# Alisah-Ozcan/HEonGPU

Measured on AMD Instinct MI355X. Metric: homomorphic mults/sec (CKKS N=2^16, L=16) + NTT GB/s vs HBM roofline, higher is better.
Workload: dtype u64

## Files before the change

### heongpu_amd/csrc/ntt.hip

```cpp
#include "ntt.hpp"
#define HEGPU_FP_TU ntt
#include "fpmod.cuh"

namespace hegpu {

#define NTT_THREADS 256

#ifdef NTT_ABLATION_HEADER
#include NTT_ABLATION_HEADER
#else
__device__ __forceinline__ u64 gld(const u64* p) { return *p; }
__device__ __forceinline__ void gst(u64* p, u64 v) { *p = v; }
#define NTT_ABLATE_BFLY(x, y, w)
#define NTT_ABLATE_FPBFLY(x, y, w)
#define NTT_ABLATE_TW(load, root0, s) (load)
#define NTT_FP_TW(t, i, c) ((t)[i])
#endif

__device__ __forceinline__ u64 csub(u64 x, u64 m) { return (x >= m) ? x - m : x; }

typedef unsigned long long u64x2_t __attribute__((ext_vector_type(2)));
struct ConstTw {
    const u64x2_t __attribute__((address_space(4)))* p;
    __device__ __forceinline__ ulonglong2 operator[](u32 i) const
    {
        const u64x2_t v = p[i];
        return make_ulonglong2(v.x, v.y);
    }
};
__device__ __forceinline__ ConstTw const_tw(const ulonglong2* t)
{
#pragma clang diagnostic push
#pragma clang diagnostic ignored "-Wold-style-cast"
    return ConstTw{(const u64x2_t __attribute__((address_space(4)))*) reinterpret_cast<const u64x2_t*>(t)};
#pragma clang diagnostic pop
}

__device__ __forceinline__ int ld_const_i32(const int* p)
{
#pragma clang diagnostic push
#pragma clang diagnostic ignored "-Wold-style-cast"
    return *(const int __attribute__((address_space(4)))*) p;
#pragma clang diagnostic pop
}
__device__ __forceinline__ Mod ld_const_mod(const Mod* p)
{
#pragma clang diagnostic push
#pragma clang diagnostic ignored "-Wold-style-cast"
    const u64 __attribute__((address_space(4)))* w = (const u64 __attribute__((address_space(4)))*) reinterpret_cast<const u64*>(p);
#pragma clang diagnostic pop
    static_assert(sizeof(Mod) == 56, "seven words");
    Mod m;
    m.q = w[0];
// ... 244 lines not shown
#pragma unroll
    for (int j = 0; j < half; j++) {
        u64 s = x[j] + x[j + half];
        u64 d = x[j] + c.q4 - x[j + half];
        x[j] = shoup_full(s, ninv, c);
        x[j + half] = shoup_full(d, w1ninv, c);
    }
}

struct PolySel {
    u64 in_off, out_off;
    int mod;
    int digit;
    int item, j;
};

__device__ __forceinline__ int udiv16(int x, unsigned magic)
{
    return magic ? (int) __umulhi((unsigned) x, magic) : x;
}

__device__ __forceinline__ PolySel select_poly(const NttArgs& a, int poly)
{
    PolySel s;
    if (a.group_span) {
        const int k = udiv16(poly, a.mg_group_span), r = poly - k * a.group_span;
        if (a.polys_per_item) {
            const int per_item = udiv16(a.polys_per_item, a.mg_mod_count);
            const int it = udiv16(r, a.mg_per_item), d = r - it * per_item;
            poly = it * a.polys_per_item + d * a.mod_count + k;
        } else {
            poly = r * a.mod_count + k;
        }
    }
    int item = 0, j = poly;
    if (a.polys_per_item) {
        item = udiv16(poly, a.mg_polys_per_item);
        j = poly - item * a.polys_per_item;
    }
    int k = j - udiv16(j, a.mg_mod_count) * a.mod_count;
    if (a.mod_order) k = a.mod_order[k];
    s.mod = a.mod_offset + k;
    u64 slot = a.poly_order ? (u64) a.poly_order[j] : (u64) j;
    s.digit = a.decomp_mods ? udiv16(j, a.mg_decomp_mods) : -1;
    u64 in_slot = a.decomp_mods ? (u64) s.digit * (a.decomp_in_mul ? a.decomp_in_mul : 1) + a.decomp_in_add : slot;
    if (a.decomp_out_mul) slot = (u64) s.digit * a.decomp_out_mul + (u64) (j - s.digit * a.decomp_mods);
    s.in_off = (u64) item * a.in_item_stride + (in_slot << a.n_power);
    s.out_off = (u64) item * a.out_item_stride + (slot << a.n_power);
    s.item = item;
    s.j = j;
    return s;
}

__device__ __forceinline__ int col_phys(int e) { return e ^ (((e >> 8) & 1) << 4); }
__device__ __forceinline__ int row_phys(int e) { return e ^ (((e >> 5) & 7) << 1); }

__device__ __forceinline__ void wave_lds_fence()
{
    __builtin_amdgcn_fence(__ATOMIC_RELEASE, "wavefront");
    __builtin_amdgcn_wave_barrier();
    __builtin_amdgcn_fence(__ATOMIC_ACQUIRE, "wavefront");
}

#define COL_LDS_ELEMS 4096
#define ROW_LDS_ELEMS 4096

__device__ __forceinline__ bool fwd_stages_lazy(const Mod& md, u64 lazy_q_max) { return md.q <= lazy_q_max; }
#define NTT_ROW_LAZY_MAX_Q 0x0666666666666666ull
__device__ __forceinline__ bool row_stages_lazy(const Mod& md, u64 lazy_q_max) { return md.q <= lazy_q_max || md.q <= NTT_ROW_LAZY_MAX_Q; }

template <int S1, bool DECOMP, bool LAZY, bool SREG = false>
__device__ __forceinline__ void fwd_col_body(const NttArgs& a, const PolySel& ps, const Mod& md, u64* lds,
                                             const u64* sreg = nullptr)
{
    constexpr int R = 1 << S1;
    constexpr int CT = 4096 / R;
    constexpr int NSA = S1 - 4;
    constexpr int RA = 1 << NSA;
    constexpr int G = 16 / RA;
    const int t = threadIdx.x;
    const QC qc = make_qc(md.q);
    const ulonglong2* __restrict__ tw = a.tw + ((u64) ps.mod << a.n_power);
    const u64* __restrict__ src = a.in + ps.in_off + blockIdx.x * CT;
    u64* __restrict__ dst = a.out + ps.out_off + blockIdx.x * CT;

    const u64 half_qP = a.half_on ? a.mods[a.half_src_mod].q : 0;
    const u64 half_hm = a.half_on ? a.half_mod[ps.mod] : 0;
    u64 x[16];
    const int col = t % CT, r1 = t / CT;
    u64 v[16];
    if constexpr (NSA > 0) {
#pragma unroll
        for (int g = 0; g < G; g++) {
            const int L = t + NTT_THREADS * g;
            const int c = L % CT, rb = L / CT;
#pragma unroll
            for (int k = 0; k < RA; k++) v[g * RA + k] = SREG ? sreg[g * RA + k] : gld(&src[(u64) (rb + 16 * k) * 256 + c]);
        }
    } else {
#pragma unroll
        for (int k = 0; k < 16; k++) v[k] = SREG ? sreg[k] : gld(&src[(u64) k * 256 + col]);
    }
    if (DECOMP && a.half_on) {
#pragma unroll
        for (int k = 0; k < 16; k++) v[k] = sub_mod(reduce64(add_mod(v[k], a.half, half_qP), md), half_hm, md.q);
    } else if (DECOMP && !LAZY && a.mods[ps.digit].q > 8 * md.q) {
#pragma unroll
        for (int k = 0; k < 16; k++) v[k] = reduce64(v[k], md);
// ... 167 lines not shown
    const u64* __restrict__ ks = ep.ks + ep.ks_item_stride * ps.item + ((u64) (part * ep.ks_part_limbs + limb) << a.n_power) + e0;
    const u64 off = ((u64) (part * ep.limbs + limb) << a.n_power);
    const bool with_ct = ep.ct && (!ep.ct_parts || part < ep.ct_parts);
    const u64* ct = with_ct ? ep.ct + ep.ct_item_stride * ps.item + off + e0 : nullptr;
    u64* out = ep.out + ep.out_item_stride * ps.item + off;
    const u64 inv = ep.inv[ps.mod];
#pragma unroll
    for (int h = 0; h < 2; h++) {
        u64 kv[8], cv[8];
#pragma unroll
        for (int k = 0; k < 8; k++) kv[k] = ks[16 * (8 * h + k)];
        if (with_ct) {
#pragma unroll
            for (int k = 0; k < 8; k++) cv[k] = ct[16 * (8 * h + k)];
        }
        u64 r[8];
#pragma unroll
        for (int k = 0; k < 8; k++)
            r[k] = mul_barrett(sub_mod(kv[k], lds[row_phys(row * 256 + i0 + 16 * (8 * h + k))], md.q), inv, md);
        if (with_ct) {
#pragma unroll
            for (int k = 0; k < 8; k++) r[k] = add_mod(cv[k], r[k], md.q);
        }
        if (ep.galois_inv) {
#pragma unroll
            for (int k = 0; k < 8; k++) {
                const u32 e = (u32) e0 + 16 * (8 * h + k);
                const u32 ex = ((2u * (__brev(e) >> (32 - a.n_power)) + 1u) * ep.galois_inv) & ((2u << a.n_power) - 1u);
                out[__brev((ex - 1u) >> 1) >> (32 - a.n_power)] = r[k];
            }
        } else {
#pragma unroll
            for (int k = 0; k < 8; k++) out[e0 + 16 * (8 * h + k)] = r[k];
        }
    }
}

template <bool LAZY>
__device__ __forceinline__ void fwd_row_body(const NttArgs& a, const PolySel& ps, const Mod& md, u64* lds)
{
    const int t = threadIdx.x;
    const QC qc = make_qc(md.q);
    const int s1 = a.n_power - 8;
    const ulonglong2* __restrict__ tw = a.tw + ((u64) ps.mod << a.n_power);
    u64* __restrict__ p = a.out + ps.out_off + (u64) blockIdx.x * 4096;

    const int row = t >> 4, i0 = t & 15;
    const u32 crow = blockIdx.x * 16 + row;
    u64 x[16];
#pragma unroll
    for (int k = 0; k < 16; k++) x[k] = gld(&p[row * 256 + i0 + 16 * k]);
    ct_radix<4, LAZY>(x, tw, (1u << s1) + crow, qc);
#pragma unroll
    for (int k = 0; k < 16; k++) lds[row_phys(row * 256 + i0 + 16 * k)] = x[k];
    wave_lds_fence();
#pragma unroll
    for (int k = 0; k < 8; k++) {
        ulonglong2 v = *reinterpret_cast<const ulonglong2*>(&lds[row_phys(row * 256 + 16 * i0 + 2 * k)]);
        x[2 * k] = v.x;
        x[2 * k + 1] = v.y;
    }
    ct_radix16_tb<LAZY>(x, a.twB + ((u64) ps.mod * (15u << (a.n_power - 4))) + ((u64) crow * 15 * 16 + i0), qc);
    if (LAZY) {
#pragma unroll
        for (int k = 0; k < 16; k++) x[k] = reduce64(x[k], md);
    } else {
#pragma unroll
        for (int k = 0; k < 16; k++) x[k] = csub(csub(csub(x[k], qc.q4), 2 * qc.q), qc.q);
    }
    wave_lds_fence();
#pragma unroll
    for (int k = 0; k < 8; k++)
        *reinterpret_cast<ulonglong2*>(&lds[row_phys(row * 256 + 16 * i0 + 2 * k)]) =
            make_ulonglong2(x[2 * k], x[2 * k + 1]);
    wave_lds_fence();
    row_store_all(a, ps, md, a.out + ps.out_off, (u64) blockIdx.x * 4096 + row * 256 + i0, lds, row, i0);
}

__device__ __forceinline__ void fwd_row_body_fp(const NttArgs& a, const PolySel& ps, const Mod& md, u64* lds)
{
    const int t = threadIdx.x;
    const FC fc = make_fc(md.q, FP_SITE(FPS_FWD_ROW, a.n_power - 12));
    const int s1 = a.n_power - 8;
    const ulonglong2* __restrict__ tw = a.tw + ((u64) ps.mod << a.n_power);
    u64* __restrict__ p = a.out + ps.out_off + (u64) blockIdx.x * 4096;

    const int row = t >> 4, i0 = t & 15;
    const u32 crow = blockIdx.x * 16 + row;
    double x[16];
#pragma unroll
    for (int k = 0; k < 16; k++) x[k] = as_f64(p[row * 256 + i0 + 16 * k]);
    fp_ct_radix<4>(x, tw, (1u << s1) + crow, fc, 0u, true);
#pragma unroll
    for (int k = 0; k < 16; k++) lds[row_phys(row * 256 + i0 + 16 * k)] = as_bits(x[k]);
    wave_lds_fence();
#pragma unroll
    for (int k = 0; k < 8; k++) {
        ulonglong2 v = *reinterpret_cast<const ulonglong2*>(&lds[row_phys(row * 256 + 16 * i0 + 2 * k)]);
        x[2 * k] = as_f64(v.x);
        x[2 * k + 1] = as_f64(v.y);
    }
    fp_ct_radix16_tb8(x, a.twB8 + ((u64) ps.mod * (15u << (a.n_power - 4))) + ((u64) crow * 15 * 16 + i0), fc);
    wave_lds_fence();
#pragma unroll
    for (int k = 0; k < 8; k++)
        *reinterpret_cast<ulonglong2*>(&lds[row_phys(row * 256 + 16 * i0 + 2 * k)]) =
            make_ulonglong2(fp_to_u64(x[2 * k]), fp_to_u64(x[2 * k + 1]));
    wave_lds_fence();
    row_store_all(a, ps, md, a.out + ps.out_off, (u64) blockIdx.x * 4096 + row * 256 + i0, lds, row, i0);
}

__global__ __launch_bounds__(NTT_THREADS) void ntt_fwd_row(NttArgs a)
{
    __shared__ __attribute__((aligned(16))) u64 lds[ROW_LDS_ELEMS];
    const PolySel ps = select_poly(a, blockIdx.y);
    if (a.skip_identity && ps.mod == ps.digit) return;
    const Mod md = a.mods[ps.mod];
    if (md.fp) fwd_row_body_fp(a, ps, md, lds);
    else if (row_stages_lazy(md, a.lazy_q_max)) fwd_row_body<true>(a, ps, md, lds);
    else fwd_row_body<false>(a, ps, md, lds);
}

template <int S1>
__device__ __forceinline__ int single_pos(int row, int col)
{
    return (row >> 4) * 4096 + row_phys((row & 15) * 256 + col);
}

template <int S1, bool FP, bool LAZY, bool DECOMP = false>
__device__ __forceinline__ void fwd_single_body(const NttArgs& a, const PolySel& ps, const Mod& md, u64* limb)
{
    constexpr int R = 1 << S1;
    constexpr int CT = 4096 / R;
    constexpr int NSA = S1 - 4;
    constexpr int RA = 1 << NSA;
    constexpr int G = 16 / RA;
    const int t = threadIdx.x, g = t >> 8, tt = t & 255;
    const QC qc = make_qc(md.q);
    const FC fc = make_fc(md.q, FP_SITE(FPS_FWD_SINGLE, S1 - 4));
    const ulonglong2* __restrict__ tw = a.tw + ((u64) ps.mod << a.n_power);
    const u64* __restrict__ src = a.in + ps.in_off + g * CT;
    const int col = tt % CT, r1 = tt / CT;
    u64 dv[DECOMP ? 16 : 1];
    double dy[(DECOMP && FP) ? 16 : 1];
    if constexpr (DECOMP) {
        if constexpr (NSA > 0) {
#pragma unroll
// ... 64 lines not shown
        } else {
#pragma unroll
            for (int k = 0; k < 16; k++) {
                if constexpr (DECOMP) x[k] = dy[k];
                else x[k] = fp_from_u64(src[(u64) k * 256 + col]);
            }
        }
        fp_ct_radix<4>(x, tw, (u32) (RA + r1), fc, FpColSched<S1>::b_before, FpColSched<S1>::b_at_end);
#pragma unroll
        for (int k = 0; k < 16; k++) limb[single_pos<S1>(16 * r1 + k, g * CT + col)] = as_bits(x[k]);
    } else {
        u64 x[16];
        if constexpr (NSA > 0) {
#pragma unroll
            for (int gi = 0; gi < G; gi++) {
                const int L = tt + 256 * gi;
                const int c = L % CT, rb = L / CT;
                u64 y[RA];
#pragma unroll
                for (int k = 0; k < RA; k++) {
                    if constexpr (DECOMP) y[k] = dv[gi * RA + k];
                    else y[k] = gld(&src[(u64) (rb + 16 * k) * 256 + c]);
                }
                ct_radix<NSA, LAZY>(y, tw, 1u, qc);
#pragma unroll
                for (int k = 0; k < RA; k++) limb[single_pos<S1>(rb + 16 * k, g * CT + c)] = y[k];
            }
            __syncthreads();
#pragma unroll
            for (int k = 0; k < 16; k++) x[k] = limb[single_pos<S1>(16 * r1 + k, g * CT + col)];
        } else {
#pragma unroll
            for (int k = 0; k < 16; k++) {
                if constexpr (DECOMP) x[k] = dv[k];
                else x[k] = src[(u64) k * 256 + col];
            }
        }
        ct_radix<4, LAZY>(x, tw, (u32) (RA + r1), qc);
#pragma unroll
        for (int k = 0; k < 16; k++) limb[single_pos<S1>(16 * r1 + k, g * CT + col)] = x[k];
    }
    __syncthreads();
    u64* lds = limb + g * 4096;
    const int row = tt >> 4, i0 = tt & 15;
    const u32 crow = g * 16 + row;
    const ulonglong2* __restrict__ tb = a.twB + ((u64) ps.mod * (15u << (a.n_power - 4))) + ((u64) crow * 15 * 16 + i0);
    u64 r[16];
    if constexpr (FP) {
        double x[16];
#pragma unroll
        for (int k = 0; k < 16; k++) x[k] = as_f64(lds[row_phys(row * 256 + i0 + 16 * k)]);
        fp_ct_radix<4>(x, tw, (1u << S1) + crow, fc, 0u, true);
#pragma unroll
        for (int k = 0; k < 16; k++) lds[row_phys(row * 256 + i0 + 16 * k)] = as_bits(x[k]);
        wave_lds_fence();
#pragma unroll
        for (int k = 0; k < 8; k++) {
            ulonglong2 v = *reinterpret_cast<const ulonglong2*>(&lds[row_phys(row * 256 + 16 * i0 + 2 * k)]);
            x[2 * k] = as_f64(v.x);
            x[2 * k + 1] = as_f64(v.y);
        }
        fp_ct_radix16_tb8(x, a.twB8 + ((u64) ps.mod * (15u << (a.n_power - 4))) + ((u64) crow * 15 * 16 + i0), fc);
#pragma unroll
        for (int k = 0; k < 16; k++) r[k] = fp_to_u64(x[k]);
    } else {
        u64 x[16];
#pragma unroll
        for (int k = 0; k < 16; k++) x[k] = lds[row_phys(row * 256 + i0 + 16 * k)];
        ct_radix<4, LAZY>(x, tw, (1u << S1) + crow, qc);
#pragma unroll
        for (int k = 0; k < 16; k++) lds[row_phys(row * 256 + i0 + 16 * k)] = x[k];
        wave_lds_fence();
#pragma unroll
        for (int k = 0; k < 8; k++) {
            ulonglong2 v = *reinterpret_cast<const ulonglong2*>(&lds[row_phys(row * 256 + 16 * i0 + 2 * k)]);
            x[2 * k] = v.x;
            x[2 * k + 1] = v.y;
        }
        ct_radix16_tb<LAZY>(x, tb, qc);
        if (LAZY) {
#pragma unroll
            for (int k = 0; k < 16; k++) r[k] = reduce64(x[k], md);
        } else {
#pragma unroll
            for (int k = 0; k < 16; k++) r[k] = csub(csub(csub(x[k], qc.q4), 2 * qc.q), qc.q);
        }
    }
    wave_lds_fence();
#pragma unroll
    for (int k = 0; k < 8; k++)
        *reinterpret_cast<ulonglong2*>(&lds[row_phys(row * 256 + 16 * i0 + 2 * k)]) = make_ulonglong2(r[2 * k], r[2 * k + 1]);
    wave_lds_fence();
    row_store_all(a, ps, md, a.out + ps.out_off, (u64) g * 4096 + row * 256 + i0, lds, row, i0);
}

template <int S1, bool DECOMP = false>
__global__ __launch_bounds__(16 << S1, 4) void ntt_fwd_single(NttArgs a)
{
    extern __shared__ __attribute__((aligned(16))) u64 limb[];
    const PolySel ps = select_poly(a, blockIdx.x);
    if (DECOMP && a.skip_identity && ps.mod == ps.digit) return;
    const Mod md = a.mods[ps.mod];
    if (md.fp) fwd_single_body<S1, true, false, DECOMP>(a, ps, md, limb);
    else if (fwd_stages_lazy(md, a.lazy_q_max)) fwd_single_body<S1, false, true, DECOMP>(a, ps, md, limb);
    else fwd_single_body<S1, false, false, DECOMP>(a, ps, md, limb);
}

__device__ __forceinline__ void acc128(u64& hi, u64& lo, u64 a, u64 b)
{
    u64 h, l;
    mul64wide(a, b, h, l);
    lo += l;
    hi += h + (lo < l);
}

template <bool LAZY>
__device__ __forceinline__ void ks_row_digit(u64 (&x)[16], const u64* __restrict__ p, u64* lds,
                                             const ulonglong2* twa, const ulonglong2* __restrict__ tb,
                                             const QC& qc, const Mod& md, int row, int i0)
{
#pragma unroll
    for (int k = 0; k < 16; k++) x[k] = gld(&p[row * 256 + i0 + 16 * k]);
#pragma unroll
    for (int s = 0; s < 4; s++) {
        const int half = 8 >> s;
#pragma unroll
        for (int b = 0; b < (1 << s); b++) {
            const ulonglong2 w = twa[((1 << s) - 1 + b) * 16 + row];
#pragma unroll
            for (int j = 0; j < half; j++) ct_bfly<LAZY>(x[b * 2 * half + j], x[b * 2 * half + j + half], w, qc);
        }
    }
#pragma unroll
    for (int k = 0; k < 16; k++) lds[row_phys(row * 256 + i0 + 16 * k)] = x[k];
    wave_lds_fence();
#pragma unroll
    for (int k = 0; k < 8; k++) {
        ulonglong2 v = *reinterpret_cast<const ulonglong2*>(&lds[row_phys(row * 256 + 16 * i0 + 2 * k)]);
        x[2 * k] = v.x;
        x[2 * k + 1] = v.y;
    }
    ct_radix16_tb<LAZY>(x, tb, qc);
    if (!LAZY) {
#pragma unroll
        for (int k = 0; k < 16; k++) x[k] = csub(csub(csub(x[k], qc.q4), 2 * qc.q), qc.q);
    }
    wave_lds_fence();
#pragma unroll
    for (int k = 0; k < 8; k++)
        *reinterpret_cast<ulonglong2*>(&lds[row_phys(row * 256 + 16 * i0 + 2 * k)]) =
            make_ulonglong2(x[2 * k], x[2 * k + 1]);
    wave_lds_fence();
#pragma unroll
    for (int k = 0; k < 16; k++) x[k] = lds[row_phys(row * 256 + i0 + 16 * k)];
    wave_lds_fence();
}

struct KsIdx { int item, tile, slot; bool valid; int d0, d1; };
__host__ __device__ __forceinline__ unsigned ks_slots(const KsMacArgs& a, int kind)
{
    const int all = a.slot_count ? a.slot_count : a.rc;
    if (a.int_slot_count <= 0 || kind == 0) return (unsigned) all;
    return kind == 1 ? (unsigned) a.int_slot_count : (unsigned) (all - a.int_slot_count);
}
template <bool SPLIT, int KIND = 0>
__device__ __forceinline__ KsIdx ks_index(const KsMacArgs& a)
{
    const unsigned b = blockIdx.x, xcd = b & 7u, j = b >> 3;
    const unsigned splits = SPLIT ? (unsigned) a.splits : 1u;
    const unsigned units = (unsigned) a.items * splits;
    const unsigned tiles = 1u << (a.n_power - 12);
    const unsigned total = ks_slots(a, KIND) * tiles * units, chunk = (total + 7u) >> 3;
    const unsigned lin = xcd * chunk + j;
    const unsigned g = lin / units, unit = lin - g * units;
    const unsigned item = SPLIT ? unit / splits : unit, sp = SPLIT ? unit - item * splits : 0u;
    const unsigned nslots = ks_slots(a, KIND), gt = g / nslots;
    KsIdx r;
    r.valid = lin < total;
    r.item = (int) item;
    r.tile = (int) gt;
    int si = (int) (g - gt * nslots);
    if (KIND == 1 && a.int_slot_count > 0) {
        si = a.int_slots[r.valid ? si : 0];
    } else {
        si += a.slot_first;
        if (KIND == 2 && a.int_slot_count > 0) {
#pragma unroll
// ... 103 lines not shown
            acc0[k] = reduce128(h0[k], l0[k], md);
            acc1[k] = reduce128(h1[k], l1[k], md);
        }
        int tt = threadIdx.x;
        asm volatile("" : "+v"(tt));
        const int trow = tt >> 4, ti0 = tt & 15;
        const u64 e0 = (u64) tile_s * 4096 + trow * 256 + ti0;
        const u64 inv = a.tail.inv[midx_s];
        const bool lazy_t = row_stages_lazy(md, a.lazy_q_max);
        const ulonglong2* __restrict__ ttb = a.twB + ((u64) midx_s * (15u << (a.n_power - 4))) + ((u64) (tile_s * 16 + trow) * 15 * 16 + ti0);
        auto part = [&](int p, const u64 (&acc)[16]) {
            u64 cv[16], x[16];
            const bool with_ct = ks_tail_ct(a, item_s, slot_s, p, e0, cv);
            const u64* pT = ks_tail_T(a, item_s, slot_s, tile_s, p);
            if (lazy_t) {
                ks_row_digit<true>(x, pT, lds, twa, ttb, qc, md, trow, ti0);
#pragma unroll
                for (int k = 0; k < 16; k++) x[k] = reduce64(x[k], md);
            } else {
                ks_row_digit<false>(x, pT, lds, twa, ttb, qc, md, trow, ti0);
            }
            ks_tail_store(a, item_s, slot_s, p, e0, md, inv, acc, x, with_ct, cv);
        };
        __builtin_amdgcn_sched_barrier(0);
        part(0, acc0);
        __builtin_amdgcn_sched_barrier(0);
        part(1, acc1);
        return;
    }
    u64* po = (SPLIT ? const_cast<u64*>(pin) + dig_off * ki.d0 - (u64) tile * 4096
                     : a.out + a.out_item_stride * item + ((u64) slot << a.n_power)) +
              (u64) tile * 4096 + row * 256 + i0;
#pragma unroll
    for (int k = 0; k < 16; k++) {
        po[16 * k] = reduce128(h0[k], l0[k], md);
        po[dig_off + 16 * k] = reduce128(h1[k], l1[k], md);
    }
    (void) n;
}

template <bool SPLIT>
__global__ __launch_bounds__(NTT_THREADS, SPLIT ? 2 : 1) void ks_row_mac(KsMacArgs a)
{
    __shared__ __attribute__((aligned(16))) u64 lds[ROW_LDS_ELEMS];
    __shared__ ulonglong2 twa[15 * 16];
    const KsIdx ki = ks_index<SPLIT, SPLIT ? 0 : 1>(a);
    if (!ki.valid) return;
    const int midx = a.mod_order ? a.mod_order[ki.slot] : ki.slot;
    const Mod md = a.mods[midx];
    if (md.fp) return;
    ks_row_mac_int_body<SPLIT>(a, ki, md, midx, lds, twa);
}

template <bool SPLIT>
__device__ __forceinline__ void ks_fp_row(double (&x)[16], const u64 (&xr)[16], const double* twl, u64* lds, const FC& fc,
                                          int s1, int row, int i0, int t)
{
    if constexpr (SPLIT) {
#pragma unroll
        for (int k = 0; k < 16; k++) x[k] = as_f64(xr[k]);
#pragma unroll
        for (int s = 0; s < 4; s++) {
            const int half = 8 >> s;
            FP_STAGE(fc, s1 + s);
#pragma unroll
            for (int b = 0; b < (1 << s); b++) {
                const double w = twl[15 * 256 + ((1 << s) - 1 + b) * 16 + row];
                const ulonglong2 wp = make_ulonglong2(as_bits(w), as_bits(w * fc.qi));
#pragma unroll
                for (int j = 0; j < half; j++) fp_ct_bfly(x[b * 2 * half + j], x[b * 2 * half + j + half], wp, fc);
            }
        }
        FP_STAGE(fc, s1 + 4);
#pragma unroll
        for (int k = 0; k < 16; k++) x[k] = fp_reduce(x[k], fc);
#pragma unroll
        for (int k = 0; k < 16; k++) lds[row_phys(row * 256 + i0 + 16 * k)] = as_bits(x[k]);
        wave_lds_fence();
#pragma unroll
        for (int k = 0; k < 8; k++) {
            ulonglong2 v = *reinterpret_cast<const ulonglong2*>(&lds[row_phys(row * 256 + 16 * i0 + 2 * k)]);
            x[2 * k] = as_f64(v.x);
            x[2 * k + 1] = as_f64(v.y);
        }
#pragma unroll
        for (int s = 0; s < 4; s++) {
            const int half = 8 >> s;
            FP_STAGE(fc, s1 + 4 + s);
#pragma unroll
            for (int b = 0; b < (1 << s); b++) {
                const double wd = twl[((1 << s) - 1 + b) * 256 + t];
                const ulonglong2 w = make_ulonglong2(as_bits(wd), as_bits(wd * fc.qi));
#pragma unroll
                for (int j = 0; j < half; j++) fp_ct_bfly(x[b * 2 * half + j], x[b * 2 * half + j + half], w, fc);
            }
        }
    } else {
        int row_o = row, t_o = t;
        asm volatile("" : "+v"(row_o), "+v"(t_o));
        const double* twa = twl + 15 * 256 + row_o;
        const double* twb = twl + t_o;
        double wn[8], wc[8];
        wc[0] = twa[0];
        wn[0] = twa[16];
        wn[1] = twa[32];
        __builtin_amdgcn_sched_barrier(0);
#pragma unroll
        for (int k = 0; k < 16; k++) x[k] = as_f64(xr[k]);
#pragma unroll
        for (int s = 0; s < 4; s++) {
            const int half = 8 >> s;
            FP_STAGE(fc, s1 + s);
            if (s > 0) {
#pragma unroll
                for (int b = 0; b < (1 << s); b++) wc[b] = wn[b];
            }
            if (s < 3) {
                if (s > 0) {
#pragma unroll
                    for (int b = 0; b < (2 << s); b++) wn[b] = twa[((2 << s) - 1 + b) * 16];
                }
            } else {
                wn[0] = twb[0];
            }
            __builtin_amdgcn_sched_barrier(0);
#pragma unroll
            for (int b = 0; b < (1 << s); b++) {
                const double w = wc[b];
                const ulonglong2 wp = make_ulonglong2(as_bits(w), as_bits(w * fc.qi));
#pragma unroll
                for (int j = 0; j < half; j++) fp_ct_bfly(x[b * 2 * half + j], x[b * 2 * half + j + half], wp, fc);
            }
        }
        FP_STAGE(fc, s1 + 4);
#pragma unroll
        for (int k = 0; k < 16; k++) x[k] = fp_reduce(x[k], fc);
#pragma unroll
        for (int k = 0; k < 16; k++) lds[row_phys(row * 256 + i0 + 16 * k)] = as_bits(x[k]);
        wave_lds_fence();
#pragma unroll
        for (int k = 0; k < 8; k++) {
            ulonglong2 v = *reinterpret_cast<const ulonglong2*>(&lds[row_phys(row * 256 + 16 * i0 + 2 * k)]);
            x[2 * k] = as_f64(v.x);
            x[2 * k + 1] = as_f64(v.y);
        }
#pragma unroll
        for (int s = 0; s < 4; s++) {
            const int half = 8 >> s;
            FP_STAGE(fc, s1 + 4 + s);
#pragma unroll
            for (int b = 0; b < (1 << s); b++) wc[b] = wn[b];
            if (s < 3) {
#pragma unroll
                for (int b = 0; b < (2 << s); b++) wn[b] = twb[((2 << s) - 1 + b) * 256];
            }
            __builtin_amdgcn_sched_barrier(0);
#pragma unroll
            for (int b = 0; b < (1 << s); b++) {
                const double wd = wc[b];
                const ulonglong2 w = make_ulonglong2(as_bits(wd), as_bits(wd * fc.qi));
#pragma unroll
                for (int j = 0; j < half; j++) fp_ct_bfly(x[b * 2 * half + j], x[b * 2 * half + j + half], w, fc);
            }
        }
    }
    wave_lds_fence();
#pragma unroll
    for (int k = 0; k < 8; k++)
        *reinterpret_cast<ulonglong2*>(&lds[row_phys(row * 256 + 16 * i0 + 2 * k)]) =
            make_ulonglong2(as_bits(x[2 * k]), as_bits(x[2 * k + 1]));
    wave_lds_fence();
#pragma unroll
    for (int k = 0; k < 16; k++) x[k] = as_f64(lds[row_phys(row * 256 + i0 + 16 * k)]);
    wave_lds_fence();
}

template <bool SPLIT, bool MD = false>
__device__ __forceinline__ void ks_row_mac_fp_body(const KsMacArgs& a, const KsIdx& ki, const Mod& md, int midx,
                                                   u64* lds, void* twbuf)
{
    const int t = threadIdx.x;
    const int item = ki.item, tile = ki.tile, slot = ki.slot;
    const FC fc = make_fc(md.q, FP_SITE(SPLIT ? FPS_KS_ROW_SPLIT : FPS_KS_ROW, a.n_power - 12));
    const int s1 = a.n_power - 8;
    const ulonglong2* __restrict__ tw = a.tw + ((u64) midx << a.n_power);
    const int row = t >> 4, i0 = t & 15;
    const u32 crow = tile * 16 + row;
    const double* __restrict__ tb8 = a.twB8 + ((u64) midx * (15u << (a.n_power - 4))) + ((u64) crow * 15 * 16 + i0);
    const u64* __restrict__ pin = a.in + a.in_item_stride * item + ((u64) slot << a.n_power) + (u64) tile * 4096;
    const u64* __restrict__ pk = a.key + ((u64) midx << a.n_power) + (u64) tile * 4096 + row * 256 + i0;
    const u64 dig_off = (u64) a.rc << a.n_power;
    const u64 key_off1 = (u64) a.key_limbs << a.n_power, key_off2 = (u64) a.key_limbs << (a.n_power + 1);

    double* twl = reinterpret_cast<double*>(twbuf);
#pragma unroll
    for (int k = 0; k < 15; k++) twl[k * 256 + t] = tb8[k * 16];
    if (i0 < 15) {
        const int s = (i0 >= 7) ? 3 : (i0 >= 3) ? 2 : (i0 >= 1) ? 1 : 0;
        const int b = i0 - ((1 << s) - 1);
        twl[15 * 256 + i0 * 16 + row] = as_f64(tw[((((u32) 1 << s1) + crow) << s) + b].x);
    }
    wave_lds_fence();

    const int item_s = MD ? __builtin_amdgcn_readfirstlane(item) : 0, slot_s = MD ? __builtin_amdgcn_readfirstlane(slot) : 0;
    const int tile_s = MD ? __builtin_amdgcn_readfirstlane(tile) : 0, midx_s = MD ? __builtin_amdgcn_readfirstlane(midx) : 0;
    double a0[16], a1[16];
#pragma unroll
    for (int k = 0; k < 16; k++) a0[k] = a1[k] = 0.0;
    int since = 0;
    for (int i = ki.d0; i < ki.d1; i++) {
        double x[16];
        const u64* p = pin + dig_off * i;
        const bool ident = a.skip_identity && i == midx;
        const u64* px = ident ? a.ident + a.ident_item_stride * item + ((u64) i << a.n_power) + (u64) tile * 4096 : p;
        u64 xr[16];
#pragma unroll
        for (int k = 0; k < 16; k++) {
            if constexpr (!SPLIT) xr[k] = __builtin_nontemporal_load(&px[row * 256 + i0 + 16 * k]);
            else xr[k] = px[row * 256 + i0 + 16 * k];
        }
        const u64* k0 = pk + key_off2 * i;
        const u64* k1 = k0 + key_off1;
        u64 kv0[16], kv1[16];
#pragma unroll
        for (int k = 0; k < 16; k++) {
            kv0[k] = k0[16 * k];
            kv1[k] = k1[16 * k];
        }
        if (ident) {
            FP_STAGE(fc, FP_STAGE_INPUT);
#pragma unroll
            for (int k = 0; k < 16; k++) x[k] = fp_reduce(fp_from_u64(xr[k]), fc);
        } else {
            ks_fp_row<SPLIT>(x, xr, twl, lds, fc, s1, row, i0, t);
        }
#pragma unroll
        for (int k = 0; k < 16; k++) {
            const double xi = x[k] * fc.qi;
            FP_STAGE(fc, FP_STAGE_PRODUCT);
            a0[k] += fp_mul(fp_from_u64(kv0[k]), x[k], xi, fc);
            a1[k] += fp_mul(fp_from_u64(kv1[k]), x[k], xi, fc);
            FP_STAGE(fc, FP_STAGE_SUMS + since);
            FP_AUDIT_VAL(fc, FPM_SUM, a0[k]);
            FP_AUDIT_VAL(fc, FPM_SUM, a1[k]);
        }
        if (++since == 3) {
            since = 0;
            FP_STAGE(fc, FP_STAGE_SUMS + 3);
#pragma unroll
            for (int k = 0; k < 16; k++) {
                a0[k] = fp_reduce(a0[k], fc);
                a1[k] = fp_reduce(a1[k], fc);
            }
        }
    }
    if constexpr (MD) {
        int tt = threadIdx.x;
        asm volatile("" : "+v"(tt));
        const int trow = tt >> 4, ti0 = tt & 15;
        const u64 e0 = (u64) tile_s * 4096 + trow * 256 + ti0;
        const Mod mds = a.mods[midx_s];
        const u64 inv = a.tail.inv[midx_s];
        auto part = [&](int p, const double (&acc)[16]) {
            const u64* pT = ks_tail_T(a, item_s, slot_s, tile_s, p);
            u64 tr[16], cv[16];
#pragma unroll
            for (int k = 0; k < 16; k++) tr[k] = __builtin_nontemporal_load(&pT[trow * 256 + ti0 + 16 * k]);
            const bool with_ct = ks_tail_ct(a, item_s, slot_s, p, e0, cv);
            double x[16];
            ks_fp_row<false>(x, tr, twl, lds, fc, s1, trow, ti0, tt);
            FP_STAGE(fc, FP_STAGE_OUT);
            u64 av[16], tv[16];
#pragma unroll
            for (int k = 0; k < 16; k++) {
                av[k] = fp_to_u64(fp_canon(acc[k], fc));
                tv[k] = fp_to_u64(fp_canon(x[k], fc));
            }
            ks_tail_store(a, item_s, slot_s, p, e0, mds, inv, av, tv, with_ct, cv);
        };
        __builtin_amdgcn_sched_barrier(0);
        part(0, a0);
        __builtin_amdgcn_sched_barrier(0);
        part(1, a1);
        return;
    }
    u64* po = (SPLIT ? const_cast<u64*>(pin) + dig_off * ki.d0 - (u64) tile * 4096
                     : a.out + a.out_item_stride * item + ((u64) slot << a.n_power)) +
              (u64) tile * 4096 + row * 256 + i0;
    FP_STAGE(fc, FP_STAGE_OUT);
#pragma unroll
    for (int k = 0; k < 16; k++) {
        if constexpr (!SPLIT) {
            __builtin_nontemporal_store(fp_to_u64(fp_canon(a0[k], fc)), &po[16 * k]);
            __builtin_nontemporal_store(fp_to_u64(fp_canon(a1[k], fc)), &po[dig_off + 16 * k]);
        } else {
            po[16 * k] = fp_to_u64(fp_canon(a0[k], fc));
            po[dig_off + 16 * k] = fp_to_u64(fp_canon(a1[k], fc));
        }
    }
}

template <bool SPLIT>
__global__ __launch_bounds__(NTT_THREADS) void ks_row_mac_fp(KsMacArgs a)
{
    __shared__ __attribute__((aligned(16))) u64 lds[ROW_LDS_ELEMS];
    __shared__ double twl[15 * 256 + 15 * 16];
    const KsIdx ki = ks_index<SPLIT, SPLIT ? 0 : 2>(a);
    if (!ki.valid) return;
    const int midx = a.mod_order ? a.mod_order[ki.slot] : ki.slot;
    const Mod md = a.mods[midx];
    if (!md.fp) return;
    ks_row_mac_fp_body<SPLIT>(a, ki, md, midx, lds, twl);
}

__global__ __launch_bounds__(NTT_THREADS) void ks_row_mac_fp_moddown(KsMacArgs a)
{
    __shared__ __attribute__((aligned(16))) u64 lds[ROW_LDS_ELEMS];
    __shared__ double twl[15 * 256 + 15 * 16];
    const KsIdx ki = ks_index<false, 2>(a);
    if (!ki.valid) return;
    const int midx = a.mod_order ? a.mod_order[ki.slot] : ki.slot;
    const Mod md = a.mods[midx];
    if (!md.fp) return;
    ks_row_mac_fp_body<false, true>(a, ki, md, midx, lds, twl);
}
__global__ __launch_bounds__(NTT_THREADS, 1) void ks_row_mac_moddown(KsMacArgs a)
{
    __shared__ __attribute__((aligned(16))) u64 lds[ROW_LDS_ELEMS];
    __shared__ ulonglong2 twa[15 * 16];
    const KsIdx ki = ks_index<false, 1>(a);
    if (!ki.valid) return;
    const int midx = a.mod_order ? a.mod_order[ki.slot] : ki.slot;
    const Mod md = a.mods[midx];
    if (md.fp) return;
    ks_row_mac_int_body<false, true>(a, ki, md, midx, lds, twa);
}
// ... 164 lines not shown
                u64 va0[4], va1[4], vb0[4], vb1[4];
#pragma unroll
                for (int k = 0; k < 4; k++) {
                    const int e = row * 256 + i0 + 16 * (k0 + k);
                    va0[k] = a0[e]; va1[k] = a1[e]; vb0[k] = b0[e]; vb1[k] = b1[e];
                }
#pragma unroll
                for (int k = 0; k < 4; k++) {
                    u64 h1, l1, h2, l2;
                    mul64wide(va0[k], vb1[k], h1, l1);
                    mul64wide(va1[k], vb0[k], h2, l2);
                    const u64 lo = l1 + l2;
                    r[k] = reduce128(h1 + h2 + (lo < l1), lo, md);
                }
            } else {
                const u64* __restrict__ pa = tensor_part == 0 ? a0 : a1;
                const u64* __restrict__ pb = tensor_part == 0 ? b0 : b1;
                u64 va[4], vb[4];
#pragma unroll
                for (int k = 0; k < 4; k++) {
                    const int e = row * 256 + i0 + 16 * (k0 + k);
                    va[k] = pa[e]; vb[k] = pb[e];
                }
#pragma unroll
                for (int k = 0; k < 4; k++) r[k] = mul_barrett(va[k], vb[k], md);
            }
#pragma unroll
            for (int k = 0; k < 4; k++) lds[row_phys(row * 256 + i0 + 16 * (k0 + k))] = r[k];
        }
    } else {
#pragma unroll
        for (int k = 0; k < 16; k++) lds[row_phys(row * 256 + i0 + 16 * k)] = gld(&src[row * 256 + i0 + 16 * k]);
    }
    wave_lds_fence();
    T x[16];
#pragma unroll
    for (int k = 0; k < 8; k++) {
        ulonglong2 v = *reinterpret_cast<const ulonglong2*>(&lds[row_phys(row * 256 + 16 * i0 + 2 * k)]);
        x[2 * k] = ar.from_canon(v.x);
        x[2 * k + 1] = ar.from_canon(v.y);
    }
    ar.radix16_tb(x, a.itwB + ((u64) mod * (15u << (a.n_power - 4))) + ((u64) crow * 15 * 16 + i0));
    wave_lds_fence();
#pragma unroll
    for (int k = 0; k < 8; k++)
        *reinterpret_cast<ulonglong2*>(&lds[row_phys(row * 256 + 16 * i0 + 2 * k)]) =
            make_ulonglong2(ar.to_bits(x[2 * k]), ar.to_bits(x[2 * k + 1]));
    wave_lds_fence();
#pragma unroll
    for (int k = 0; k < 16; k++) x[k] = ar.from_bits(lds[row_phys(row * 256 + i0 + 16 * k)]);
    ar.template radix<4>(x, tw, (1u << s1) + crow);
    if constexpr (TO_LDS) {
#pragma unroll
        for (int k = 0; k < 16; k++) lds[row_phys(row * 256 + i0 + 16 * k)] = ar.to_bits(x[k]);
    } else {
#pragma unroll
        for (int k = 0; k < 16; k++) gst(&dst[row * 256 + i0 + 16 * k], ar.to_bits(x[k]));
    }
}

struct InvEpi {
    const u64* last;
    const u64* ct;
    u64* out;
    Mod md;
    u64 half, qP, hm, inv;
    int galois, n_power;
    bool pre;
};
__device__ __forceinline__ bool inv_epi_setup(const NttArgs& a, const PolySel& ps, InvEpi& e, bool& skip)
{
    skip = false;
    if (!a.iepi.on) return false;
    const NttInvEpilogue& ep = a.iepi;
    const int pc = ep.p_count ? ep.p_count : 1;
    const int part = udiv16(ps.j, ep.mg_slots), limb = ps.j - part * (ep.limbs + pc);
    if (limb >= ep.limbs) { skip = true; return true; }
    const u64 item_in = a.out_item_stride * ps.item;
    const u64 off = (u64) (part * ep.limbs + limb) << a.n_power;
    e.pre = ep.u != nullptr;
    e.last = e.pre ? ep.u + ep.u_item_stride * ps.item + off
                   : a.out + item_in + ((u64) (part * (ep.limbs + 1) + ep.limbs) << a.n_power);
    e.ct = (ep.ct && part < ep.add_parts) ? ep.ct + ep.ct_item_stride * ps.item + off : nullptr;
    e.out = ep.out + ep.out_item_stride * ps.item + off;
    e.md = a.mods[ps.mod];
    e.half = ep.half;
    e.qP = a.mods[ep.p_mod].q;
    e.hm = e.pre ? 0 : ep.half_mod[limb];
    e.inv = ep.inv[limb];
    e.galois = ep.galois_elt;
    e.n_power = a.n_power;
    return true;
}
template <int CNT, bool EPI, typename POS>
__device__ __forceinline__ void inv_store(const InvEpi& epr, u64* __restrict__ p, u32 e0, POS pos, const u64 (&o)[CNT])
{
    if constexpr (!EPI) {
#pragma unroll
        for (int k = 0; k < CNT; k++) gst(&p[pos(k)], o[k]);
        return;
    }
    const InvEpi* ep = &epr;
    u64 lv[CNT], cv[CNT], r[CNT];
#pragma unroll
    for (int k = 0; k < CNT; k++) lv[k] = ep->last[e0 + pos(k)];
    if (ep->ct) {
#pragma unroll
// ... 512 lines not shown
```

Baseline: 8312.

## Retune row LDS swizzle and prefetch next keyswitch digit across row NTT

Changes the row LDS swizzle to XOR with bits 4-7 instead of 5-7 and reorders the scalar LDS stores so interleaved k indices hit different banks, aiming to cut bank conflicts in the row transposes. In the non-split keyswitch MAC loop it software-pipelines global loads: the next digit's input (or the tail T for the MD path) is loaded after the current row NTT, and the key loads are injected mid-NTT through a hook placed between sched_barriers. This hides HBM latency behind compute at the cost of extra live registers, which may reduce occupancy.

```diff
diff --git a/heongpu_amd/csrc/lds_swizzle.hpp b/heongpu_amd/csrc/lds_swizzle.hpp
--- /dev/null
+++ b/heongpu_amd/csrc/lds_swizzle.hpp
@@ -0,0 +1,19 @@
+#pragma once
+
+#ifndef HG_HD
+#if defined(__HIPCC__)
+#define HG_HD __host__ __device__ __forceinline__
+#else
+#define HG_HD inline
+#endif
+#endif
+
+namespace hegpu {
+
+HG_HD int col_phys(int e) { return e ^ (((e >> 8) & 1) << 4); }
+
+HG_HD int row_phys(int e) { return e ^ (((e >> 4) & 15) << 1); }
+
+HG_HD int row_store_order(int j) { return (j >> 1) | ((j & 1) << 3); }
+
+}
diff --git a/heongpu_amd/csrc/ntt.hip b/heongpu_amd/csrc/ntt.hip
--- a/heongpu_amd/csrc/ntt.hip
+++ b/heongpu_amd/csrc/ntt.hip
@@ -1,4 +1,5 @@
 #include "ntt.hpp"
+#include "lds_swizzle.hpp"
 #define HEGPU_FP_TU ntt
 #include "fpmod.cuh"
 
@@ -349,8 +350,6 @@
     return s;
 }
 
-__device__ __forceinline__ int col_phys(int e) { return e ^ (((e >> 8) & 1) << 4); }
-__device__ __forceinline__ int row_phys(int e) { return e ^ (((e >> 5) & 7) << 1); }
 
 __device__ __forceinline__ void wave_lds_fence()
 {
@@ -624,7 +623,7 @@
     for (int k = 0; k < 16; k++) x[k] = gld(&p[row * 256 + i0 + 16 * k]);
     ct_radix<4, LAZY>(x, tw, (1u << s1) + crow, qc);
 #pragma unroll
-    for (int k = 0; k < 16; k++) lds[row_phys(row * 256 + i0 + 16 * k)] = x[k];
+    for (int j = 0; j < 16; j++) { const int k = row_store_order(j); lds[row_phys(row * 256 + i0 + 16 * k)] = x[k]; }
     wave_lds_fence();
 #pragma unroll
     for (int k = 0; k < 8; k++) {
@@ -664,7 +663,7 @@
     for (int k = 0; k < 16; k++) x[k] = as_f64(p[row * 256 + i0 + 16 * k]);
     fp_ct_radix<4>(x, tw, (1u << s1) + crow, fc, 0u, true);
 #pragma unroll
-    for (int k = 0; k < 16; k++) lds[row_phys(row * 256 + i0 + 16 * k)] = as_bits(x[k]);
+    for (int j = 0; j < 16; j++) { const int k = row_store_order(j); lds[row_phys(row * 256 + i0 + 16 * k)] = as_bits(x[k]); }
     wave_lds_fence();
 #pragma unroll
     for (int k = 0; k < 8; k++) {
@@ -835,7 +834,7 @@
         for (int k = 0; k < 16; k++) x[k] = as_f64(lds[row_phys(row * 256 + i0 + 16 * k)]);
         fp_ct_radix<4>(x, tw, (1u << S1) + crow, fc, 0u, true);
 #pragma unroll
-        for (int k = 0; k < 16; k++) lds[row_phys(row * 256 + i0 + 16 * k)] = as_bits(x[k]);
+        for (int j = 0; j < 16; j++) { const int k = row_store_order(j); lds[row_phys(row * 256 + i0 + 16 * k)] = as_bits(x[k]); }
         wave_lds_fence();
 #pragma unroll
         for (int k = 0; k < 8; k++) {
@@ -852,7 +851,7 @@
         for (int k = 0; k < 16; k++) x[k] = lds[row_phys(row * 256 + i0 + 16 * k)];
         ct_radix<4, LAZY>(x, tw, (1u << S1) + crow, qc);
 #pragma unroll
-        for (int k = 0; k < 16; k++) lds[row_phys(row * 256 + i0 + 16 * k)] = x[k];
+        for (int j = 0; j < 16; j++) { const int k = row_store_order(j); lds[row_phys(row * 256 + i0 + 16 * k)] = x[k]; }
         wave_lds_fence();
 #pragma unroll
         for (int k = 0; k < 8; k++) {
@@ -915,7 +914,7 @@
         }
     }
 #pragma unroll
-    for (int k = 0; k < 16; k++) lds[row_phys(row * 256 + i0 + 16 * k)] = x[k];
+    for (int j = 0; j < 16; j++) { const int k = row_store_order(j); lds[row_phys(row * 256 + i0 + 16 * k)] = x[k]; }
     wave_lds_fence();
 #pragma unroll
     for (int k = 0; k < 8; k++) {
@@ -1125,9 +1124,10 @@
     ks_row_mac_int_body<SPLIT>(a, ki, md, midx, lds, twa);
 }
 
-template <bool SPLIT>
+struct KsNoHook { __device__ void operator()() const {} };
+template <bool SPLIT, typename MID = KsNoHook>
 __device__ __forceinline__ void ks_fp_row(double (&x)[16], const u64 (&xr)[16], const double* twl, u64* lds, const FC& fc,
-                                          int s1, int row, int i0, int t)
+                                          int s1, int row, int i0, int t, MID mid = MID())
 {
     if constexpr (SPLIT) {
 #pragma unroll
@@ -1148,7 +1148,7 @@
 #pragma unroll
         for (int k = 0; k < 16; k++) x[k] = fp_reduce(x[k], fc);
 #pragma unroll
-        for (int k = 0; k < 16; k++) lds[row_phys(row * 256 + i0 + 16 * k)] = as_bits(x[k]);
+        for (int j = 0; j < 16; j++) { const int k = row_store_order(j); lds[row_phys(row * 256 + i0 + 16 * k)] = as_bits(x[k]); }
         wave_lds_fence();
 #pragma unroll
         for (int k = 0; k < 8; k++) {
@@ -1209,8 +1209,11 @@
 #pragma unroll
         for (int k = 0; k < 16; k++) x[k] = fp_reduce(x[k], fc);
 #pragma unroll
-        for (int k = 0; k < 16; k++) lds[row_phys(row * 256 + i0 + 16 * k)] = as_bits(x[k]);
+        for (int j = 0; j < 16; j++) { const int k = row_store_order(j); lds[row_phys(row * 256 + i0 + 16 * k)] = as_bits(x[k]); }
         wave_lds_fence();
+        __builtin_amdgcn_sched_barrier(0);
+        mid();
+        __builtin_amdgcn_sched_barrier(0);
 #pragma unroll
         for (int k = 0; k < 8; k++) {
             ulonglong2 v = *reinterpret_cast<const ulonglong2*>(&lds[row_phys(row * 256 + 16 * i0 + 2 * k)]);
@@ -1281,31 +1284,58 @@
 #pragma unroll
     for (int k = 0; k < 16; k++) a0[k] = a1[k] = 0.0;
     int since = 0;
+    auto load_digit = [&](int d, u64 (&v)[16]) {
+        const bool id = a.skip_identity && d == midx;
+        const u64* px = id ? a.ident + a.ident_item_stride * item + ((u64) d << a.n_power) + (u64) tile * 4096
+                           : pin + dig_off * d;
+#pragma unroll
+        for (int k = 0; k < 16; k++) {
+            if constexpr (!SPLIT) v[k] = __builtin_nontemporal_load(&px[row * 256 + i0 + 16 * k]);
+            else v[k] = px[row * 256 + i0 + 16 * k];
+        }
+    };
+    u64 xr[16];
+    auto load_next = [&](int d) {
+        if (d < ki.d1) {
+            load_digit(d, xr);
+        } else if constexpr (MD) {
+            const u64* pT = ks_tail_T(a, item_s, slot_s, tile_s, 0);
+#pragma unroll
+            for (int k = 0; k < 16; k++) xr[k] = __builtin_nontemporal_load(&pT[row * 256 + i0 + 16 * k]);
+        }
+    };
+    if constexpr (!SPLIT) load_next(ki.d0);
     for (int i = ki.d0; i < ki.d1; i++) {
         double x[16];
-        const u64* p = pin + dig_off * i;
         const bool ident = a.skip_identity && i == midx;
-        const u64* px = ident ? a.ident + a.ident_item_stride * item + ((u64) i << a.n_power) + (u64) tile * 4096 : p;
-        u64 xr[16];
-#pragma unroll
-        for (int k = 0; k < 16; k++) {
-            if constexpr (!SPLIT) xr[k] = __builtin_nontemporal_load(&px[row * 256 + i0 + 16 * k]);
-            else xr[k] = px[row * 256 + i0 + 16 * k];
-        }
         const u64* k0 = pk + key_off2 * i;
         const u64* k1 = k0 + key_off1;
         u64 kv0[16], kv1[16];
-#pragma unroll
-        for (int k = 0; k < 16; k++) {
-            kv0[k] = k0[16 * k];
-            kv1[k] = k1[16 * k];
+        auto load_key = [&]() {
+#pragma unroll
+            for (int k = 0; k < 16; k++) {
+                kv0[k] = k0[16 * k];
+                kv1[k] = k1[16 * k];
+            }
+        };
+        if constexpr (SPLIT) {
+            load_digit(i, xr);
+            load_key();
         }
         if (ident) {
+            if constexpr (!SPLIT) load_key();
             FP_STAGE(fc, FP_STAGE_INPUT);
 #pragma unroll
             for (int k = 0; k < 16; k++) x[k] = fp_reduce(fp_from_u64(xr[k]), fc);
+        } else if constexpr (SPLIT) {
+            ks_fp_row<SPLIT>(x, xr, twl, lds, fc, s1, row, i0, t);
         } else {
-            ks_fp_row<SPLIT>(x, xr, twl, lds, fc, s1, row, i0, t);
+            ks_fp_row<SPLIT>(x, xr, twl, lds, fc, s1, row, i0, t, load_key);
+        }
+        if constexpr (!SPLIT) {
+            __builtin_amdgcn_sched_barrier(0);
+            load_next(i + 1);
+            __builtin_amdgcn_sched_barrier(0);
         }
 #pragma unroll
         for (int k = 0; k < 16; k++) {
@@ -1334,11 +1364,8 @@
         const u64 e0 = (u64) tile_s * 4096 + trow * 256 + ti0;
         const Mod mds = a.mods[midx_s];
         const u64 inv = a.tail.inv[midx_s];
-        auto part = [&](int p, const double (&acc)[16]) {
-            const u64* pT = ks_tail_T(a, item_s, slot_s, tile_s, p);
-            u64 tr[16], cv[16];
-#pragma unroll
-            for (int k = 0; k < 16; k++) tr[k] = __builtin_nontemporal_load(&pT[trow * 256 + ti0 + 16 * k]);
+        auto part = [&](int p, const double (&acc)[16], const u64 (&tr)[16]) {
+            u64 cv[16];
             const bool with_ct = ks_tail_ct(a, item_s, slot_s, p, e0, cv);
             double x[16];
             ks_fp_row<false>(x, tr, twl, lds, fc, s1, trow, ti0, tt);
@@ -1352,9 +1379,12 @@
             ks_tail_store(a, item_s, slot_s, p, e0, mds, inv, av, tv, with_ct, cv);
         };
         __builtin_amdgcn_sched_barrier(0);
-        part(0, a0);
+        part(0, a0, xr);
         __builtin_amdgcn_sched_barrier(0);
-        part(1, a1);
+        const u64* pT1 = ks_tail_T(a, item_s, slot_s, tile_s, 1);
+#pragma unroll
+        for (int k = 0; k < 16; k++) xr[k] = __builtin_nontemporal_load(&pT1[trow * 256 + ti0 + 16 * k]);
+        part(1, a1, xr);
         return;
     }
     u64* po = (SPLIT ? const_cast<u64*>(pin) + dig_off * ki.d0 - (u64) tile * 4096
@@ -1625,7 +1655,7 @@
     ar.template radix<4>(x, tw, (1u << s1) + crow);
     if constexpr (TO_LDS) {
 #pragma unroll
-        for (int k = 0; k < 16; k++) lds[row_phys(row * 256 + i0 + 16 * k)] = ar.to_bits(x[k]);
+        for (int j = 0; j < 16; j++) { const int k = row_store_order(j); lds[row_phys(row * 256 + i0 + 16 * k)] = ar.to_bits(x[k]); }
     } else {
 #pragma unroll
         for (int k = 0; k < 16; k++) gst(&dst[row * 256 + i0 + 16 * k], ar.to_bits(x[k]));
```

After: 8349 (median of 6 runs). Within noise of the previous version (+0.4%).
